# lreithmayr/ORB_SLAM2_2021

Hardware: AMD Instinct MI355X
Metric: frames/sec (ORB extract+match) on 1241×376, 1/2/4/8 MI355X; % HBM roofline (higher is better)
Workload: dtype u8

## Files before the change

orb_slam2_2021_amd/csrc/orbfe_extract.hip:

```cpp
#include <hip/hip_runtime.h>

#include <algorithm>
#include <atomic>
#include <chrono>
#include <condition_variable>
#include <functional>
#include <thread>
#include <cfloat>
#include <cmath>
#include <cstdio>
#include <cstdlib>
#include <cstring>
#include <mutex>
#include <string>
#include <type_traits>
#include <vector>

#include "../../include/orbfe.h"
#include "../../include/orbfe_debug.h"
#include "orb_pattern31.inc"
#include "orbfe_device.h"
#include "orbfe_internal.h"
#include "orbfe_ktimer.h"

// ... 1004 lines not shown
        const int m = mp[0];
        const int mn = max(max(max(max((int)mp[-mw - 1], (int)mp[-mw]), max((int)mp[-mw + 1], (int)mp[-1])),
                               max(max((int)mp[1], (int)mp[mw - 1]), (int)mp[mw])), (int)mp[mw + 1]);
        sc = m - 1;
        keep = m >= max(t + 1, 2) && m > mn;
      }
      const uint64_t bal = wave_ballot(keep);
      if (keep) out[count + prefix_in_wave(bal)] = pack_key(cc + 3 + cd.ox, rr + 3 + cd.oy, sc);
      count += __popcll(bal);
    }
    if (count > 0) break;
  }
  if (lane == 0) *cnt_out = count;
}

#define OCT_MISC_SCALAR 16
#define OCT_MISC_INTS 32
struct ONode {
  int16_t x0, y0, x1, y1;
  int32_t begin, count, seq, flags;
};


__device__ __forceinline__ int child_of(uint32_t key, int mx, int my) {
  return (key_x(key) >= mx ? 1 : 0) | (key_y(key) >= my ? 2 : 0);
}

__device__ __forceinline__ int4 wave_child_counts(const ONode& nd, const uint32_t* ka, const uint32_t* kb) {
  const uint32_t* src = (nd.flags & 1) ? kb : ka;
  const int mx = nd.x0 + ((nd.x1 - nd.x0 + 1) >> 1), my = nd.y0 + ((nd.y1 - nd.y0 + 1) >> 1);
  int c0 = 0, c1 = 0, c2 = 0, c3 = 0;
  for (int i0 = 0; i0 < nd.count; i0 += 64) {
    const int i = i0 + lane_id();
    const int ch = i < nd.count ? child_of(src[nd.begin + i], mx, my) : -1;
    c0 += __popcll(wave_ballot(ch == 0));
    c1 += __popcll(wave_ballot(ch == 1));
    c2 += __popcll(wave_ballot(ch == 2));
    c3 += __popcll(wave_ballot(ch == 3));
  }
  return make_int4(c0, c1, c2, c3);
}

__device__ __forceinline__ void wave_child_partition(const ONode& nd, int4 cnt, uint32_t* ka, uint32_t* kb) {
  const uint32_t* src = (nd.flags & 1) ? kb : ka;
  uint32_t* dst = (nd.flags & 1) ? ka : kb;
  const int mx = nd.x0 + ((nd.x1 - nd.x0 + 1) >> 1), my = nd.y0 + ((nd.y1 - nd.y0 + 1) >> 1);
  int o0 = nd.begin, o1 = o0 + cnt.x, o2 = o1 + cnt.y, o3 = o2 + cnt.z;
  for (int i0 = 0; i0 < nd.count; i0 += 64) {
    const int i = i0 + lane_id();
    uint32_t key = 0;
    int ch = -1;
    if (i < nd.count) {
      key = src[nd.begin + i];
      ch = child_of(key, mx, my);
    }
    const uint64_t b0 = wave_ballot(ch == 0), b1 = wave_ballot(ch == 1), b2 = wave_ballot(ch == 2),
                   b3 = wave_ballot(ch == 3);
    if (ch == 0) dst[o0 + prefix_in_wave(b0)] = key;
    if (ch == 1) dst[o1 + prefix_in_wave(b1)] = key;
    if (ch == 2) dst[o2 + prefix_in_wave(b2)] = key;
    if (ch == 3) dst[o3 + prefix_in_wave(b3)] = key;
    o0 += __popcll(b0);
    o1 += __popcll(b1);
    o2 += __popcll(b2);
    o3 += __popcll(b3);
  }
}

#ifndef OCT_SMALL
#define OCT_SMALL 48
#endif
#define OCT_SMALL_MAX 128
__device__ __forceinline__ int4 serial_child_counts(const ONode& nd, const uint32_t* ka, const uint32_t* kb) {
  const uint32_t* src = ((nd.flags & 1) ? kb : ka) + nd.begin;
  const int mx = nd.x0 + ((nd.x1 - nd.x0 + 1) >> 1), my = nd.y0 + ((nd.y1 - nd.y0 + 1) >> 1);
  uint32_t c = 0;
  if (nd.count <= 16) {
    uint32_t key[16];
#pragma unroll
    for (int j = 0; j < 16; j++) key[j] = j < nd.count ? src[j] : 0u;
#pragma unroll
    for (int j = 0; j < 16; j++)
      if (j < nd.count) c += 1u << (8 * child_of(key[j], mx, my));
    return make_int4((int)(c & 255u), (int)((c >> 8) & 255u), (int)((c >> 16) & 255u), (int)(c >> 24));
  }
  int i = 0;
  for (; i + 4 <= nd.count; i += 4) {
    const uint32_t k0 = src[i], k1 = src[i + 1], k2 = src[i + 2], k3 = src[i + 3];
    c += (1u << (8 * child_of(k0, mx, my))) + (1u << (8 * child_of(k1, mx, my))) +
         (1u << (8 * child_of(k2, mx, my))) + (1u << (8 * child_of(k3, mx, my)));
  }
  for (; i < nd.count; i++) c += 1u << (8 * child_of(src[i], mx, my));
  return make_int4((int)(c & 255u), (int)((c >> 8) & 255u), (int)((c >> 16) & 255u), (int)(c >> 24));
}

__device__ __forceinline__ void serial_child_partition(const ONode& nd, int4 cnt, uint32_t* ka, uint32_t* kb) {
  const uint32_t* src = ((nd.flags & 1) ? kb : ka) + nd.begin;
  uint32_t* dst = ((nd.flags & 1) ? ka : kb) + nd.begin;
  const int mx = nd.x0 + ((nd.x1 - nd.x0 + 1) >> 1), my = nd.y0 + ((nd.y1 - nd.y0 + 1) >> 1);
  uint32_t o = ((uint32_t)cnt.x << 8) | ((uint32_t)(cnt.x + cnt.y) << 16) | ((uint32_t)(cnt.x + cnt.y + cnt.z) << 24);
  auto put = [&](uint32_t key) {
    const int sh = 8 * child_of(key, mx, my);
    dst[(o >> sh) & 255u] = key;
    o += 1u << sh;
  };
  if (nd.count <= 16) {
    uint32_t key[16];
#pragma unroll
    for (int j = 0; j < 16; j++) key[j] = j < nd.count ? src[j] : 0u;
#pragma unroll
    for (int j = 0; j < 16; j++)
      if (j < nd.count) put(key[j]);
    return;
  }
  int i = 0;
  for (; i + 4 <= nd.count; i += 4) {
    const uint32_t k0 = src[i], k1 = src[i + 1], k2 = src[i + 2], k3 = src[i + 3];
    put(k0);
    put(k1);
    put(k2);
    put(k3);
  }
  for (; i < nd.count; i++) put(src[i]);
}

#define OCT_WJ 16
#define OCT_SJ 16
__device__ __forceinline__ int4 wave_child_split(const ONode& nd, uint32_t* ka, uint32_t* kb) {
  if (nd.count > 64 * OCT_WJ) {
    const int4 c4 = wave_child_counts(nd, ka, kb);
    wave_child_partition(nd, c4, ka, kb);
    return c4;
  }
  const uint32_t* src = ((nd.flags & 1) ? kb : ka) + nd.begin;
  uint32_t* dst = ((nd.flags & 1) ? ka : kb) + nd.begin;
  const int mx = nd.x0 + ((nd.x1 - nd.x0 + 1) >> 1), my = nd.y0 + ((nd.y1 - nd.y0 + 1) >> 1);
  const int lane = lane_id();
  uint32_t key[OCT_WJ];
  int ch[OCT_WJ];
#pragma unroll
  for (int j = 0; j < OCT_WJ; j++) {
    const int i = 64 * j + lane;
    key[j] = i < nd.count ? src[i] : 0u;
  }
  int c0 = 0, c1 = 0, c2 = 0, c3 = 0;
#pragma unroll
  for (int j = 0; j < OCT_WJ; j++) {
    if (64 * j >= nd.count) break;
    ch[j] = 64 * j + lane < nd.count ? child_of(key[j], mx, my) : -1;
    c0 += __popcll(wave_ballot(ch[j] == 0));
    c1 += __popcll(wave_ballot(ch[j] == 1));
    c2 += __popcll(wave_ballot(ch[j] == 2));
    c3 += __popcll(wave_ballot(ch[j] == 3));
  }
  int o0 = 0, o1 = c0, o2 = c0 + c1, o3 = c0 + c1 + c2;
#pragma unroll
  for (int j = 0; j < OCT_WJ; j++) {
    if (64 * j >= nd.count) break;
    const uint64_t b0 = wave_ballot(ch[j] == 0), b1 = wave_ballot(ch[j] == 1), b2 = wave_ballot(ch[j] == 2),
                   b3 = wave_ballot(ch[j] == 3);
    if (ch[j] == 0) dst[o0 + prefix_in_wave(b0)] = key[j];
    if (ch[j] == 1) dst[o1 + prefix_in_wave(b1)] = key[j];
    if (ch[j] == 2) dst[o2 + prefix_in_wave(b2)] = key[j];
    if (ch[j] == 3) dst[o3 + prefix_in_wave(b3)] = key[j];
    o0 += __popcll(b0);
    o1 += __popcll(b1);
    o2 += __popcll(b2);
    o3 += __popcll(b3);
  }
  return make_int4(c0, c1, c2, c3);
}

__device__ __forceinline__ int4 serial_child_split(const ONode& nd, uint32_t* ka, uint32_t* kb) {
  if (nd.count > OCT_SJ) {
    const int4 c4 = serial_child_counts(nd, ka, kb);
    serial_child_partition(nd, c4, ka, kb);
    return c4;
  }
  const uint32_t* src = ((nd.flags & 1) ? kb : ka) + nd.begin;
  uint32_t* dst = ((nd.flags & 1) ? ka : kb) + nd.begin;
  const int mx = nd.x0 + ((nd.x1 - nd.x0 + 1) >> 1), my = nd.y0 + ((nd.y1 - nd.y0 + 1) >> 1);
  uint32_t key[OCT_SJ];
#pragma unroll
  for (int j = 0; j < OCT_SJ; j++) key[j] = j < nd.count ? src[j] : 0u;
  uint32_t c = 0;
#pragma unroll
  for (int j = 0; j < OCT_SJ; j++)
    if (j < nd.count) c += 1u << (8 * child_of(key[j], mx, my));
  const uint32_t c0 = c & 255u, c1 = (c >> 8) & 255u, c2 = (c >> 16) & 255u;
  uint32_t o = (c0 << 8) | ((c0 + c1) << 16) | ((c0 + c1 + c2) << 24);
#pragma unroll
  for (int j = 0; j < OCT_SJ; j++)
    if (j < nd.count) {
      const int sh = 8 * child_of(key[j], mx, my);
      dst[(o >> sh) & 255u] = key[j];
      o += 1u << sh;
    }
  return make_int4((int)c0, (int)c1, (int)c2, (int)(c >> 24));
}

__device__ __forceinline__ ONode make_child(const ONode& p, int c, int begin, int count, int seq) {
  const int mx = p.x0 + ((p.x1 - p.x0 + 1) >> 1), my = p.y0 + ((p.y1 - p.y0 + 1) >> 1);
  ONode n;
  n.x0 = (int16_t)((c & 1) ? mx : p.x0);
  n.x1 = (int16_t)((c & 1) ? p.x1 : mx);
  n.y0 = (int16_t)((c & 2) ? my : p.y0);
  n.y1 = (int16_t)((c & 2) ? p.y1 : my);
  n.begin = begin;
  n.count = count;
  n.seq = seq;
  n.flags = ((p.flags & 1) ^ 1) | (count > 1 ? 2 : 0);
  return n;
}

__device__ __forceinline__ int nonempty4(int4 c) {
  return (c.x > 0) + (c.y > 0) + (c.z > 0) + (c.w > 0);
}
__device__ __forceinline__ int multi4(int4 c) {
  return (c.x > 1) + (c.y > 1) + (c.z > 1) + (c.w > 1);
}
__device__ __forceinline__ int comp4(int4 c, int k) {
  return k == 0 ? c.x : k == 1 ? c.y : k == 2 ? c.z : c.w;
}

template <int NW, typename Idx, typename F>
__device__ __forceinline__ void for_big_nodes(const ONode* L, int m, int small, Idx idx, F f) {
  const int w = wave_id(), lane = lane_id();
  int ord = 0;
  for (int c0 = 0; c0 < m; c0 += 64) {
    const int p = c0 + lane;
    const bool big = p < m && L[idx(p)].count > small;
    uint64_t bal = wave_ballot(big);
    while (bal) {
      const int b = __builtin_ctzll(bal);
      bal &= bal - 1;
      if (ord % NW == w) f(c0 + b);
      ord++;
    }
  }
}

#ifdef ORBFE_OCT_PROF
__device__ unsigned long long g_oct_prof[64 * 16 * 16];
#define OCT_MARK(k, v) \
  do { if (threadIdx.x == 0 && blockIdx.y < 64 && l < 16) g_oct_prof[(blockIdx.y * 16 + l) * 16 + (k)] = (v); } while (0)
#else
#define OCT_MARK(k, v) do { } while (0)
#endif
#ifdef ORBFE_OCT_PROF_PASS
#define OCT_RMARK(k, v) do { } while (0)
#define OCT_PMARK(k, v) do { if (n_passes == ORBFE_OCT_PROF_PASS) OCT_MARK(k, v); } while (0)
#else
#define OCT_RMARK(k, v) OCT_MARK(k, v)
#define OCT_PMARK(k, v) do { } while (0)
#endif

template <bool LDSK, int NT>
__device__ __forceinline__ void octree_run(const ExtractArgs& a, uint8_t* smem, int l, int n, uint32_t* ka,
                                           uint32_t* kb) {
  constexpr int NW = NT / 64;
  const int img = blockIdx.y;
  const int t = threadIdx.x, w = wave_id(), lane = lane_id();
  const int NC = a.node_cap, SC = a.sort_cap, SA = a.scan_cap;
  const int SMALL = a.oct_small;
  ONode* nodes0 = reinterpret_cast<ONode*>(smem);
  ONode* nodes1 = nodes0 + NC;
  int4* cc = reinterpret_cast<int4*>(nodes1 + NC);
  int* sa = reinterpret_cast<int*>(cc + NC);
  int* sb = sa + SA;
  int* sx = sb + SA;
  unsigned long long* sk = reinterpret_cast<unsigned long long*>(sx + SA);
  int* misc = reinterpret_cast<int*>(sk + SC);
  const LevelDesc ld = a.levels[l];
  const int N = ld.budget;
  const uint32_t* cand = a.cand + (long long)img * a.cand_stride;
  uint32_t* out = a.lvlkeys + (long long)img * a.lvlkey_stride + ld.key_begin;
  int32_t* out_n = a.lvlcnt + (long long)img * a.nlevels + l;

  const int ncells = ld.ncells;
  for (int c = t; c < ncells; c += NT) {
    const int b0 = sa[c], cnt = (c + 1 < ncells ? sa[c + 1] : n) - b0;
    const uint32_t* src = cand + sx[c];
    int k = 0;
    for (; k + 4 <= cnt; k += 4) {
      const uint32_t v0 = src[k], v1 = src[k + 1], v2 = src[k + 2], v3 = src[k + 3];
      ka[b0 + k] = v0;
      ka[b0 + k + 1] = v1;
      ka[b0 + k + 2] = v2;
      ka[b0 + k + 3] = v3;
    }
    for (; k < cnt; k++) ka[b0 + k] = src[k];
  }
  __syncthreads();
  OCT_MARK(2, wall_clock64());

  const int nini = ld.nini;
  const float hx = ld.hx;
  auto ini_node = [&](uint32_t key) -> int {
    const int x = key_x(key);
    if (nini > 8) return (int)((float)x / hx);
    int b = 0;
#pragma unroll
    for (int k = 1; k < 8; k++) b += (k < nini && x >= ld.ini_thr[k]) ? 1 : 0;
    return b;
  };
  int* bcnt = reinterpret_cast<int*>(sk);
  int* boff = bcnt + NW * nini;
  const int R = ((n + NW - 1) / NW + 63) & ~63;
  const int wbeg = min(w * R, n), wend = min(wbeg + R, n);
  constexpr int INI_J = NT >= 1024 ? 8 : 24;
  const bool cached = wend - wbeg <= 64 * INI_J;
  uint32_t kr[INI_J];
  int br[INI_J];
  const int nj = (wend - wbeg + 63) >> 6;
  if (cached) {
#pragma unroll
    for (int j = 0; j < INI_J; j++) br[j] = -1;
    if (nini <= 8) {
#pragma unroll
      for (int j = 0; j < INI_J; j++) {
        if (j >= nj) break;
        const int i = wbeg + 64 * j + lane;
        kr[j] = i < wend ? ka[i] : 0u;
        const int x = key_x(kr[j]);
        int b = 0;
#pragma unroll
// ... 84 lines not shown
    }
  }
  __syncthreads();
  if (t == 0) {
    int S = 0, run = 0;
    for (int b = 0; b < nini; b++) {
      const int cnt = sb[b];
      if (cnt > 0) {
        ONode nd;
        nd.x0 = (int16_t)(int)(hx * (float)b);
        nd.x1 = (int16_t)(int)(hx * (float)(b + 1));
        nd.y0 = 0;
        nd.y1 = (int16_t)ld.rel_h;
        nd.begin = run;
        nd.count = cnt;
        nd.seq = b;
        nd.flags = 1;
        nodes0[S++] = nd;
      }
      run += cnt;
    }
    misc[OCT_MISC_SCALAR] = S;
  }
  __syncthreads();

  int S = misc[OCT_MISC_SCALAR];
  int cur = 0;
  bool refine = false;
  OCT_MARK(3, wall_clock64());
  int n_passes = 0, n_rounds = 0;
  for (int iter = 0; iter < 4 * NC + 64; iter++) {
    ONode* Lc = cur ? nodes1 : nodes0;
    ONode* Ln = cur ? nodes0 : nodes1;
    const int prevS = S;
    if (!refine) {
      n_passes++;
#ifdef ORBFE_OCT_PROF_PASS
      if (n_passes == ORBFE_OCT_PROF_PASS) OCT_MARK(14, wall_clock64());
#endif
      for (int i = t; i < S; i += NT) {
        const ONode nd = Lc[i];
        if (nd.count > SMALL) continue;
        const bool par = nd.count > 1;
        const int4 c4 = par ? serial_child_split(nd, ka, kb) : make_int4(0, 0, 0, 0);
        if (par) cc[i] = c4;
        sa[i] = par ? nonempty4(c4) : 0;
        sb[i] = par ? 0 : 1;
        sx[i] = par ? multi4(c4) : 0;
      }
      OCT_PMARK(8, wall_clock64());
#ifdef ORBFE_OCT_PROF_PASS
      unsigned long long split_cyc = 0, split_n = 0;
#endif
      for_big_nodes<NW>(Lc, S, SMALL, [](int p) { return p; }, [&](int i) {
#ifdef ORBFE_OCT_PROF_PASS
        const unsigned long long c0 = clock64();
        const int4 c4 = wave_child_split(Lc[i], ka, kb);
        split_cyc += clock64() - c0;
        split_n += (unsigned long long)Lc[i].count << 16 | 1ull;
#else
        const int4 c4 = wave_child_split(Lc[i], ka, kb);
#endif
        if (lane == 0) {
          cc[i] = c4;
          sa[i] = nonempty4(c4);
          sb[i] = 0;
          sx[i] = multi4(c4);
        }
      });
      OCT_PMARK(9, wall_clock64());
#ifdef ORBFE_OCT_PROF_PASS
      OCT_PMARK(12, split_cyc);
      OCT_PMARK(13, split_n);
#endif
      __syncthreads();
      OCT_PMARK(10, wall_clock64());
#ifndef ORBFE_OCT_PROF_PASS
      if (n_passes == 1) OCT_MARK(14, wall_clock64());
#endif
      const int3 tot3 = block_scan_excl3_n<NT>(sa, sb, sx, S, reinterpret_cast<int*>(sk));
#ifndef ORBFE_OCT_PROF_PASS
      if (n_passes == 1) OCT_MARK(15, wall_clock64());
#endif
      OCT_PMARK(11, wall_clock64());
      const int T = tot3.x, NP = tot3.y, nexp = tot3.z;
      for (int i = t; i < S; i += NT) {
        const ONode nd = Lc[i];
        if (nd.count > 1) {
          const int4 c4 = cc[i];
          int e = sa[i], off = nd.begin;
          for (int k = 0; k < 4; k++) {
            const int ck = comp4(c4, k);
            if (ck > 0) {
              Ln[T - 1 - e] = make_child(nd, k, off, ck, e);
              e++;
            }
            off += ck;
          }
        } else {
          ONode m = nd;
          m.flags &= 1;
          Ln[T + sb[i]] = m;
        }
      }
      S = T + NP;
      cur ^= 1;
      __syncthreads();
#ifdef ORBFE_OCT_PROF_PASS
      if (n_passes == ORBFE_OCT_PROF_PASS) OCT_MARK(15, wall_clock64());
#endif
      if (S >= N || S == prevS) break;
      if (S + nexp * 3 > N) refine = true;
    } else {
      if (n_rounds++ == 0) OCT_MARK(4, wall_clock64());
      for (int i = t; i < S; i += NT) sa[i] = (Lc[i].flags & 2) ? 1 : 0;
      __syncthreads();
      const int nR = block_scan_excl_n<NT>(sa, S, misc);
      if (n_rounds == 1) OCT_RMARK(8, wall_clock64());
      int P2 = 1;
      while (P2 < nR) P2 <<= 1;
      if (nR > 1024) {
        for (int i = t; i < P2; i += NT) sk[i] = 0ull;
        __syncthreads();
      }
      for (int i = t; i < S; i += NT) {
        const ONode nd = Lc[i];
        if (nd.flags & 2)
          sk[sa[i]] = ((unsigned long long)nd.count << 40) | ((unsigned long long)nd.seq << 20) |
                      (unsigned long long)i;
      }
      __syncthreads();
      if (nR <= 1024) {
        constexpr int RP = (1024 + NT - 1) / NT;
        unsigned long long kk[RP];
        int rk[RP];
#pragma unroll
        for (int r = 0; r < RP; r++) {
          const int k = t + NT * r;
          kk[r] = k < nR ? sk[k] : 0ull;
          rk[r] = 0;
        }
        const int per = (nR + NT - 1) / NT;
        int j = 0;
// ... 25 lines not shown
            for (int pidx = t; pidx < (P2 >> 1); pidx += NT) {
              const int i = ((pidx & ~(j - 1)) << 1) | (pidx & (j - 1)), ixj = i + j;
              const unsigned long long x = sk[i], y = sk[ixj];
              if ((i & k) == 0 ? (x < y) : (x > y)) {
                sk[i] = y;
                sk[ixj] = x;
              }
            }
            __syncthreads();
          }
        }
      }
      if (n_rounds == 1) OCT_RMARK(9, wall_clock64());
      for (int k = t; k < nR; k += NT) {
        const ONode nd = Lc[(int)(sk[k] & 0xfffffull)];
        if (nd.count <= SMALL) cc[k] = serial_child_counts(nd, ka, kb);
      }
      for_big_nodes<NW>(Lc, nR, SMALL, [&](int k) { return (int)(sk[k] & 0xfffffull); }, [&](int k) {
        const int4 c4 = wave_child_counts(Lc[(int)(sk[k] & 0xfffffull)], ka, kb);
        if (lane == 0) cc[k] = c4;
      });
      __syncthreads();
      if (n_rounds == 1) OCT_RMARK(10, wall_clock64());
      for (int k = t; k < nR; k += NT) sa[k] = nonempty4(cc[k]) - 1;
      if (t == 0) misc[OCT_MISC_SCALAR + 1] = nR;
      __syncthreads();
      block_scan_excl_n<NT>(sa, nR, misc);
      for (int k = t; k < nR; k += NT) {
        const int incl = sa[k] + nonempty4(cc[k]) - 1;
        if (prevS + incl >= N) atomicMin(&misc[OCT_MISC_SCALAR + 1], k + 1);
      }
      __syncthreads();
      const int nproc = misc[OCT_MISC_SCALAR + 1];
      if (n_rounds == 1) OCT_RMARK(11, wall_clock64());
      for (int i = t; i < S; i += NT) sb[i] = -1;
      __syncthreads();
      for (int k = t; k < nproc; k += NT) sb[(int)(sk[k] & 0xfffffull)] = k;
      __syncthreads();
      for (int k = t; k < nproc; k += NT) {
        const ONode nd = Lc[(int)(sk[k] & 0xfffffull)];
        if (nd.count <= SMALL) serial_child_partition(nd, cc[k], ka, kb);
      }
      for_big_nodes<NW>(Lc, nproc, SMALL, [&](int k) { return (int)(sk[k] & 0xfffffull); }, [&](int k) {
        wave_child_partition(Lc[(int)(sk[k] & 0xfffffull)], cc[k], ka, kb);
      });
      for (int k = t; k < nR; k += NT) sx[k] = k < nproc ? nonempty4(cc[k]) : 0;
      __syncthreads();
      if (n_rounds == 1) OCT_RMARK(12, wall_clock64());
      const int T = block_scan_excl_n<NT>(sx, nR, misc);
      for (int i = t; i < S; i += NT) sa[i] = sb[i] < 0 ? 1 : 0;
      __syncthreads();
      const int NK = block_scan_excl_n<NT>(sa, S, misc);
      for (int i = t; i < S; i += NT) {
        const ONode nd = Lc[i];
        const int k = sb[i];
        if (k >= 0) {
          const int4 c4 = cc[k];
          int e = sx[k], off = nd.begin;
          for (int c = 0; c < 4; c++) {
            const int ck = comp4(c4, c);
            if (ck > 0) {
              Ln[T - 1 - e] = make_child(nd, c, off, ck, e);
              e++;
            }
            off += ck;
          }
        } else {
          ONode m = nd;
          m.flags &= 1;
          Ln[T + sa[i]] = m;
        }
      }
      S = T + NK;
      cur ^= 1;
      __syncthreads();
      if (n_rounds == 1) OCT_RMARK(13, wall_clock64());
      if (S >= N || S == prevS) break;
    }
  }

  OCT_MARK(5, wall_clock64());
  if (n_rounds == 0) OCT_MARK(4, wall_clock64());
  ONode* Lf = cur ? nodes1 : nodes0;
  for (int i = t; i < S; i += NT) {
    const ONode nd = Lf[i];
    const uint32_t* src = (nd.flags & 1) ? kb : ka;
    uint32_t best = src[nd.begin];
    for (int k = 1; k < nd.count; k++) {
      const uint32_t key = src[nd.begin + k];
      if (key_s(key) > key_s(best)) best = key;
    }
    out[i] = pack_key(key_x(best) + 16, key_y(best) + 16, key_s(best));
  }
  if (t == 0) *out_n = S;
#ifdef ORBFE_OCT_PROF
  __syncthreads();
  OCT_MARK(6, wall_clock64());
  OCT_MARK(7, (unsigned long long)n | ((unsigned long long)n_passes << 24) | ((unsigned long long)n_rounds << 32) |
                  ((unsigned long long)S << 48));
#endif
}


template <int NT>
__global__ __launch_bounds__(NT) void k_octree(ExtractArgs a, int l0) {
  extern __shared__ __attribute__((aligned(16))) uint8_t smem[];
  const int l = l0 + blockIdx.x, img = blockIdx.y, t = threadIdx.x;
  const int NC = a.node_cap, SC = a.sort_cap, SA = a.scan_cap;
  int* sa = reinterpret_cast<int*>(smem + (sizeof(ONode) * 2 + sizeof(int4)) * NC);
  int* sx = sa + 2 * SA;
  int* misc = reinterpret_cast<int*>(reinterpret_cast<unsigned long long*>(sx + SA) + SC);
  uint32_t* lds_keys = reinterpret_cast<uint32_t*>(misc + OCT_MISC_INTS);
  OCT_MARK(0, wall_clock64());
  const LevelDesc ld = a.levels[l];
  const int32_t* ccount = a.cellcnt + (long long)img * a.ncells + ld.cell_begin;
  for (int c = t; c < ld.ncells; c += NT) {
    sa[c] = ccount[c];
    sx[c] = a.cells[ld.cell_begin + c].slot;
  }
  __syncthreads();
  const int n = block_scan_excl_n<NT>(sa, ld.ncells, misc);
  OCT_MARK(1, wall_clock64());
  if (n == 0) {
    if (t == 0) a.lvlcnt[(long long)img * a.nlevels + l] = 0;
    return;
  }
  if (n <= a.key_lds_cap) {
    octree_run<true, NT>(a, smem, l, n, lds_keys, lds_keys + a.key_lds_cap);
  } else {
    octree_run<false, NT>(a, smem, l, n, a.keys_a + (long long)img * a.keyscr_stride + ld.cand_begin,
                      a.keys_b + (long long)img * a.keyscr_stride + ld.cand_begin);
  }
}

#define BS_W 248
#define BS_H 16
__device__ __forceinline__ int reflect101(int i, int n) {
  return i < 0 ? -i : (i >= n ? 2 * n - 2 - i : i);
}

__device__ __forceinline__ uint32_t from_left(uint32_t v) {
  return (uint32_t)__builtin_amdgcn_mov_dpp((int)v, 0x138, 0xf, 0xf, true);
}
__device__ __forceinline__ uint32_t from_right(uint32_t v) {
  return (uint32_t)__builtin_amdgcn_mov_dpp((int)v, 0x130, 0xf, 0xf, true);
}
// ... 786 lines not shown
    }
  }
  return ORBFE_OK;
}

static OctPlan octree_plan(const std::vector<LevelDesc>& lv, int l0, int l1, int budget_kb, int key_cap_override) {
  OctPlan p;
  if (l1 <= l0) return p;
  int ncap = 0, mc = 0, mini = 0;
  for (int l = l0; l < l1; l++) {
    ncap = std::max(ncap, lv[l].key_cap + 4);
    mc = std::max(mc, lv[l].ncells);
    mini = std::max(mini, lv[l].nini);
  }
  int sc = 1;
  while (sc < std::max(std::max(ncap, 16 * mini), 24)) sc <<= 1;
  p.node_cap = ncap;
  p.sort_cap = sc;
  p.scan_cap = (std::max(ncap, mc) + 3) & ~3;
  const size_t fixed = sizeof(ONode) * 2 * ncap + sizeof(int4) * ncap + sizeof(int) * 3 * p.scan_cap +
                       sizeof(unsigned long long) * sc + sizeof(int) * OCT_MISC_INTS;
  const size_t budget = (size_t)budget_kb * 1024;
  p.key_lds_cap = fixed < budget ? (int)((budget - fixed) / 8) & ~63 : 0;
  if (key_cap_override >= 0) p.key_lds_cap = std::min(p.key_lds_cap, key_cap_override);
  p.lds = fixed + sizeof(uint32_t) * 2 * (size_t)p.key_lds_cap;
  return p;
}

static void free_batch(orbfe_extractor* h) {
  if (h->hpyr_pending) {
    hipEventSynchronize(h->ev_hpyr);
    h->hpyr_pending = false;
  }
  drop_graphs(h);
  hipFree(h->d_pyr);
  hipFree(h->d_blur);
  hipFree(h->d_cand);
  hipFree(h->d_cellcnt);
  hipFree(h->d_keys_a);
  hipFree(h->d_keys_b);
// ... 243 lines not shown
    hipEvent_t e = nullptr;
    ORBFE_HIP_CHECK(hipEventCreateWithFlags(&e, kForkJoinEvent));
    h->ev_lvl.push_back(e);
  }
  hipStreamCaptureStatus cs = hipStreamCaptureStatusNone;
  if (!h->use_graphs || !st || h->side_ext || orbfe_kt::g_on.load(std::memory_order_relaxed) ||
      hipStreamIsCapturing(st, &cs) != hipSuccess || cs != hipStreamCaptureStatusNone)
    return launch_extract(h, n, d_imgs, img_stride, pitch, d_kps, d_desc, cap, d_counts, st, i0);
  const hipStream_t side = h->inline_side ? st : (h->side_ext ? h->side_ext : h->side);
  const std::vector<uintptr_t> key = {
      (uintptr_t)n, (uintptr_t)d_imgs, (uintptr_t)img_stride, (uintptr_t)pitch, (uintptr_t)d_kps,
      (uintptr_t)d_desc, (uintptr_t)cap, (uintptr_t)d_counts, (uintptr_t)st, (uintptr_t)i0, (uintptr_t)side,
      (uintptr_t)h->rows, (uintptr_t)h->cols, (uintptr_t)h->geom_mode, (uintptr_t)h->d_levels,
      (uintptr_t)h->d_pyr, (uintptr_t)h->d_blur, (uintptr_t)h->d_cand, (uintptr_t)h->d_cellcnt,
      (uintptr_t)h->d_keys_a, (uintptr_t)h->d_keys_b, (uintptr_t)h->d_lvlkeys, (uintptr_t)h->d_lvlcnt,
      (uintptr_t)h->key_lds_cap, (uintptr_t)h->octree_split, (uintptr_t)(h->oct_hi_kb * 1024 + h->oct_lo_kb), (uintptr_t)h->device_call, (uintptr_t)(h->fast_wpb_side * 16 + h->fast_wpb_main), (uintptr_t)h->fast_side_levels, (uintptr_t)h->fast_side_merge, (uintptr_t)h->input_l0, (uintptr_t)h->inline_side, (uintptr_t)(h->oct_threads_small * 4096 + h->oct_threads_batch), (uintptr_t)h->pyr_small.d_tiles, (uintptr_t)h->pyr_batch.d_tiles,
      (uintptr_t)h->blur_mode};
  h->graph_clock++;
  hipGraphExec_t exec = nullptr;
  for (auto& e : h->graphs)
    if (e.key == key) {
      exec = e.exec;
      e.used = h->graph_clock;
      h->graph_hits++;
      break;
    }
  if (!exec) {
    hipGraph_t g = nullptr;
    ORBFE_HIP_CHECK(hipStreamBeginCapture(st, hipStreamCaptureModeThreadLocal));
    const int r = launch_extract(h, n, d_imgs, img_stride, pitch, d_kps, d_desc, cap, d_counts, st, i0);
    const hipError_t ee = hipStreamEndCapture(st, &g);
// ... 936 lines not shown
  h->pyr_tiles_small[0] = small_tx;
  h->pyr_tiles_small[1] = small_ty;
  h->pyr_tiles_batch[0] = batch_tx;
  h->pyr_tiles_batch[1] = batch_ty;
  h->rows = h->cols = -1;
  drop_graphs(h);
  return ORBFE_OK;
}

extern "C" int orbfe_debug_set_octree_threads(orbfe_extractor* h, int small_calls, int batches) {
  auto ok = [](int t) { return t == 256 || t == 512 || t == 1024; };
  if (!h || !ok(small_calls) || !ok(batches))
    return orbfe_set_error(ORBFE_ERR_ARG, "orbfe_debug_set_octree_threads: 256, 512 or 1024");
  h->oct_threads_small = small_calls;
  h->oct_threads_batch = batches;
  return ORBFE_OK;
}

extern "C" int orbfe_debug_set_octree_threads_l0(orbfe_extractor* h, int threads) {
  if (!h || !(threads == 0 || threads == 256 || threads == 512 || threads == 1024))
    return orbfe_set_error(ORBFE_ERR_ARG, "orbfe_debug_set_octree_threads_l0: 0, 256, 512 or 1024");
  h->oct_threads_l0 = threads;
  return ORBFE_OK;
}

extern "C" int orbfe_debug_set_octree_serial(orbfe_extractor* h, int small_calls, int batches) {
  if (!h || small_calls < 1 || small_calls > OCT_SMALL_MAX || batches < 1 || batches > OCT_SMALL_MAX)
    return orbfe_set_error(ORBFE_ERR_ARG, "orbfe_debug_set_octree_serial: 1 .. 128 keys");
  h->oct_small_small = small_calls;
  h->oct_small_batch = batches;
  drop_graphs(h);
  return ORBFE_OK;
}

extern "C" int orbfe_debug_set_latency_schedule(orbfe_extractor* h, int k) {
  if (!h) return orbfe_set_error(ORBFE_ERR_ARG, "orbfe_debug_set_latency_schedule: null handle");
  h->lat_sched = k > 0 ? k : 0;
// ... 43 lines not shown
```

Baseline: 87000.

## Partition octree keys in place with a single LDS key buffer

The octree split now partitions keys in place within one buffer instead of ping-ponging between two buffers. Large nodes stage through a global scratch buffer and copy back. Node structs drop their seq/flags fields, and child counts are packed into 64-bit words. The sort keys alias the next node list, and a new 16-lane group split handles mid-sized nodes. The aim is to halve the LDS needed for keys so more levels keep their keys on-chip, and to spread mid-size node work across lanes. The cost is an extra copy-back for big nodes and more complex LDS aliasing.

```diff
diff --git a/orb_slam2_2021_amd/csrc/orbfe_extract.hip b/orb_slam2_2021_amd/csrc/orbfe_extract.hip
--- a/orb_slam2_2021_amd/csrc/orbfe_extract.hip
+++ b/orb_slam2_2021_amd/csrc/orbfe_extract.hip
@@ -1042,25 +1042,55 @@
   if (lane == 0) *cnt_out = count;
 }
 
-#define OCT_MISC_SCALAR 16
-#define OCT_MISC_INTS 32
+#define OCT_MISC_SCALAR 48
+#define OCT_MISC_INTS 64
 struct ONode {
   int16_t x0, y0, x1, y1;
-  int32_t begin, count, seq, flags;
+  int32_t begin, count;
 };
 
+__device__ __forceinline__ unsigned long long pack_cc(int4 c) {
+  return (unsigned long long)c.x | ((unsigned long long)c.y << 21) | ((unsigned long long)c.z << 42);
+}
+__device__ __forceinline__ int4 unpack_cc(unsigned long long v, int count) {
+  const int x = (int)(v & 0x1fffffull), y = (int)((v >> 21) & 0x1fffffull), z = (int)(v >> 42);
+  return make_int4(x, y, z, count - x - y - z);
+}
+
+struct OctLds {
+  ONode *nodes0, *nodes1;
+  unsigned long long* cc;
+  int *sa, *sb, *sx, *misc;
+  uint32_t* keys;
+};
+__host__ __device__ __forceinline__ size_t oct_list_bytes(int node_cap, int sort_cap) {
+  const size_t nb = sizeof(ONode) * (size_t)node_cap, sb = sizeof(unsigned long long) * (size_t)sort_cap;
+  return ((nb > sb ? nb : sb) + 15) & ~(size_t)15;
+}
+__device__ __forceinline__ OctLds oct_lds(uint8_t* smem, int NC, int SC, int SA) {
+  OctLds o;
+  const size_t lb = oct_list_bytes(NC, SC);
+  o.nodes0 = reinterpret_cast<ONode*>(smem);
+  o.nodes1 = reinterpret_cast<ONode*>(smem + lb);
+  o.cc = reinterpret_cast<unsigned long long*>(smem + 2 * lb);
+  o.sa = reinterpret_cast<int*>(o.cc + NC);
+  o.sb = o.sa + SA;
+  o.sx = o.sb + SA;
+  o.misc = o.sx + SA;
+  o.keys = reinterpret_cast<uint32_t*>(o.misc + OCT_MISC_INTS);
+  return o;
+}
 
 __device__ __forceinline__ int child_of(uint32_t key, int mx, int my) {
   return (key_x(key) >= mx ? 1 : 0) | (key_y(key) >= my ? 2 : 0);
 }
 
-__device__ __forceinline__ int4 wave_child_counts(const ONode& nd, const uint32_t* ka, const uint32_t* kb) {
-  const uint32_t* src = (nd.flags & 1) ? kb : ka;
+__device__ __forceinline__ int4 wave_child_counts(const ONode& nd, const uint32_t* k) {
   const int mx = nd.x0 + ((nd.x1 - nd.x0 + 1) >> 1), my = nd.y0 + ((nd.y1 - nd.y0 + 1) >> 1);
   int c0 = 0, c1 = 0, c2 = 0, c3 = 0;
   for (int i0 = 0; i0 < nd.count; i0 += 64) {
     const int i = i0 + lane_id();
-    const int ch = i < nd.count ? child_of(src[nd.begin + i], mx, my) : -1;
+    const int ch = i < nd.count ? child_of(k[nd.begin + i], mx, my) : -1;
     c0 += __popcll(wave_ballot(ch == 0));
     c1 += __popcll(wave_ballot(ch == 1));
     c2 += __popcll(wave_ballot(ch == 2));
@@ -1069,9 +1099,7 @@
   return make_int4(c0, c1, c2, c3);
 }
 
-__device__ __forceinline__ void wave_child_partition(const ONode& nd, int4 cnt, uint32_t* ka, uint32_t* kb) {
-  const uint32_t* src = (nd.flags & 1) ? kb : ka;
-  uint32_t* dst = (nd.flags & 1) ? ka : kb;
+__device__ __forceinline__ void wave_child_partition_staged(const ONode& nd, int4 cnt, uint32_t* k, uint32_t* g) {
   const int mx = nd.x0 + ((nd.x1 - nd.x0 + 1) >> 1), my = nd.y0 + ((nd.y1 - nd.y0 + 1) >> 1);
   int o0 = nd.begin, o1 = o0 + cnt.x, o2 = o1 + cnt.y, o3 = o2 + cnt.z;
   for (int i0 = 0; i0 < nd.count; i0 += 64) {
@@ -1079,28 +1107,40 @@
     uint32_t key = 0;
     int ch = -1;
     if (i < nd.count) {
-      key = src[nd.begin + i];
+      key = k[nd.begin + i];
       ch = child_of(key, mx, my);
     }
     const uint64_t b0 = wave_ballot(ch == 0), b1 = wave_ballot(ch == 1), b2 = wave_ballot(ch == 2),
                    b3 = wave_ballot(ch == 3);
-    if (ch == 0) dst[o0 + prefix_in_wave(b0)] = key;
-    if (ch == 1) dst[o1 + prefix_in_wave(b1)] = key;
-    if (ch == 2) dst[o2 + prefix_in_wave(b2)] = key;
-    if (ch == 3) dst[o3 + prefix_in_wave(b3)] = key;
+    if (ch == 0) g[o0 + prefix_in_wave(b0)] = key;
+    if (ch == 1) g[o1 + prefix_in_wave(b1)] = key;
+    if (ch == 2) g[o2 + prefix_in_wave(b2)] = key;
+    if (ch == 3) g[o3 + prefix_in_wave(b3)] = key;
     o0 += __popcll(b0);
     o1 += __popcll(b1);
     o2 += __popcll(b2);
     o3 += __popcll(b3);
   }
+  __threadfence_block();
+  __builtin_amdgcn_wave_barrier();
+  int i = lane_id();
+  for (; i + 192 < nd.count; i += 256) {
+    const uint32_t v0 = g[nd.begin + i], v1 = g[nd.begin + i + 64], v2 = g[nd.begin + i + 128],
+                   v3 = g[nd.begin + i + 192];
+    k[nd.begin + i] = v0;
+    k[nd.begin + i + 64] = v1;
+    k[nd.begin + i + 128] = v2;
+    k[nd.begin + i + 192] = v3;
+  }
+  for (; i < nd.count; i += 64) k[nd.begin + i] = g[nd.begin + i];
 }
 
 #ifndef OCT_SMALL
 #define OCT_SMALL 48
 #endif
 #define OCT_SMALL_MAX 128
-__device__ __forceinline__ int4 serial_child_counts(const ONode& nd, const uint32_t* ka, const uint32_t* kb) {
-  const uint32_t* src = ((nd.flags & 1) ? kb : ka) + nd.begin;
+__device__ __forceinline__ int4 serial_child_counts(const ONode& nd, const uint32_t* k) {
+  const uint32_t* src = k + nd.begin;
   const int mx = nd.x0 + ((nd.x1 - nd.x0 + 1) >> 1), my = nd.y0 + ((nd.y1 - nd.y0 + 1) >> 1);
   uint32_t c = 0;
   if (nd.count <= 16) {
@@ -1122,46 +1162,16 @@
   return make_int4((int)(c & 255u), (int)((c >> 8) & 255u), (int)((c >> 16) & 255u), (int)(c >> 24));
 }
 
-__device__ __forceinline__ void serial_child_partition(const ONode& nd, int4 cnt, uint32_t* ka, uint32_t* kb) {
-  const uint32_t* src = ((nd.flags & 1) ? kb : ka) + nd.begin;
-  uint32_t* dst = ((nd.flags & 1) ? ka : kb) + nd.begin;
-  const int mx = nd.x0 + ((nd.x1 - nd.x0 + 1) >> 1), my = nd.y0 + ((nd.y1 - nd.y0 + 1) >> 1);
-  uint32_t o = ((uint32_t)cnt.x << 8) | ((uint32_t)(cnt.x + cnt.y) << 16) | ((uint32_t)(cnt.x + cnt.y + cnt.z) << 24);
-  auto put = [&](uint32_t key) {
-    const int sh = 8 * child_of(key, mx, my);
-    dst[(o >> sh) & 255u] = key;
-    o += 1u << sh;
-  };
-  if (nd.count <= 16) {
-    uint32_t key[16];
-#pragma unroll
-    for (int j = 0; j < 16; j++) key[j] = j < nd.count ? src[j] : 0u;
-#pragma unroll
-    for (int j = 0; j < 16; j++)
-      if (j < nd.count) put(key[j]);
-    return;
-  }
-  int i = 0;
-  for (; i + 4 <= nd.count; i += 4) {
-    const uint32_t k0 = src[i], k1 = src[i + 1], k2 = src[i + 2], k3 = src[i + 3];
-    put(k0);
-    put(k1);
-    put(k2);
-    put(k3);
-  }
-  for (; i < nd.count; i++) put(src[i]);
-}
-
 #define OCT_WJ 16
+#define OCT_GJ 8
 #define OCT_SJ 16
-__device__ __forceinline__ int4 wave_child_split(const ONode& nd, uint32_t* ka, uint32_t* kb) {
+__device__ __forceinline__ int4 wave_child_split(const ONode& nd, uint32_t* k, uint32_t* g) {
   if (nd.count > 64 * OCT_WJ) {
-    const int4 c4 = wave_child_counts(nd, ka, kb);
-    wave_child_partition(nd, c4, ka, kb);
+    const int4 c4 = wave_child_counts(nd, k);
+    wave_child_partition_staged(nd, c4, k, g);
     return c4;
   }
-  const uint32_t* src = ((nd.flags & 1) ? kb : ka) + nd.begin;
-  uint32_t* dst = ((nd.flags & 1) ? ka : kb) + nd.begin;
+  uint32_t* seg = k + nd.begin;
   const int mx = nd.x0 + ((nd.x1 - nd.x0 + 1) >> 1), my = nd.y0 + ((nd.y1 - nd.y0 + 1) >> 1);
   const int lane = lane_id();
   uint32_t key[OCT_WJ];
@@ -1169,7 +1179,7 @@
 #pragma unroll
   for (int j = 0; j < OCT_WJ; j++) {
     const int i = 64 * j + lane;
-    key[j] = i < nd.count ? src[i] : 0u;
+    key[j] = i < nd.count ? seg[i] : 0u;
   }
   int c0 = 0, c1 = 0, c2 = 0, c3 = 0;
 #pragma unroll
@@ -1187,10 +1197,10 @@
     if (64 * j >= nd.count) break;
     const uint64_t b0 = wave_ballot(ch[j] == 0), b1 = wave_ballot(ch[j] == 1), b2 = wave_ballot(ch[j] == 2),
                    b3 = wave_ballot(ch[j] == 3);
-    if (ch[j] == 0) dst[o0 + prefix_in_wave(b0)] = key[j];
-    if (ch[j] == 1) dst[o1 + prefix_in_wave(b1)] = key[j];
-    if (ch[j] == 2) dst[o2 + prefix_in_wave(b2)] = key[j];
-    if (ch[j] == 3) dst[o3 + prefix_in_wave(b3)] = key[j];
+    if (ch[j] == 0) seg[o0 + prefix_in_wave(b0)] = key[j];
+    if (ch[j] == 1) seg[o1 + prefix_in_wave(b1)] = key[j];
+    if (ch[j] == 2) seg[o2 + prefix_in_wave(b2)] = key[j];
+    if (ch[j] == 3) seg[o3 + prefix_in_wave(b3)] = key[j];
     o0 += __popcll(b0);
     o1 += __popcll(b1);
     o2 += __popcll(b2);
@@ -1199,18 +1209,55 @@
   return make_int4(c0, c1, c2, c3);
 }
 
-__device__ __forceinline__ int4 serial_child_split(const ONode& nd, uint32_t* ka, uint32_t* kb) {
-  if (nd.count > OCT_SJ) {
-    const int4 c4 = serial_child_counts(nd, ka, kb);
-    serial_child_partition(nd, c4, ka, kb);
-    return c4;
-  }
-  const uint32_t* src = ((nd.flags & 1) ? kb : ka) + nd.begin;
-  uint32_t* dst = ((nd.flags & 1) ? ka : kb) + nd.begin;
+__device__ __forceinline__ int4 group_child_split(const ONode& nd, bool on, uint32_t* k) {
+  const int lane = lane_id(), gl = lane & 15, gsh = lane & 48;
+  const int count = on ? nd.count : 0;
+  uint32_t* seg = k + nd.begin;
+  const int mx = nd.x0 + ((nd.x1 - nd.x0 + 1) >> 1), my = nd.y0 + ((nd.y1 - nd.y0 + 1) >> 1);
+  uint32_t key[OCT_GJ];
+  int ch[OCT_GJ];
+#pragma unroll
+  for (int j = 0; j < OCT_GJ; j++) {
+    const int i = 16 * j + gl;
+    key[j] = i < count ? seg[i] : 0u;
+    ch[j] = i < count ? child_of(key[j], mx, my) : -1;
+  }
+  const uint32_t below = (1u << gl) - 1u;
+  int c0 = 0, c1 = 0, c2 = 0, c3 = 0;
+#pragma unroll
+  for (int j = 0; j < OCT_GJ; j++) {
+    if (wave_ballot(16 * j < count) == 0) break;
+    c0 += __popc((uint32_t)(wave_ballot(ch[j] == 0) >> gsh) & 0xffffu);
+    c1 += __popc((uint32_t)(wave_ballot(ch[j] == 1) >> gsh) & 0xffffu);
+    c2 += __popc((uint32_t)(wave_ballot(ch[j] == 2) >> gsh) & 0xffffu);
+    c3 += __popc((uint32_t)(wave_ballot(ch[j] == 3) >> gsh) & 0xffffu);
+  }
+  int o0 = 0, o1 = c0, o2 = c0 + c1, o3 = c0 + c1 + c2;
+#pragma unroll
+  for (int j = 0; j < OCT_GJ; j++) {
+    if (wave_ballot(16 * j < count) == 0) break;
+    const uint32_t b0 = (uint32_t)(wave_ballot(ch[j] == 0) >> gsh) & 0xffffu,
+                   b1 = (uint32_t)(wave_ballot(ch[j] == 1) >> gsh) & 0xffffu,
+                   b2 = (uint32_t)(wave_ballot(ch[j] == 2) >> gsh) & 0xffffu,
+                   b3 = (uint32_t)(wave_ballot(ch[j] == 3) >> gsh) & 0xffffu;
+    if (ch[j] == 0) seg[o0 + __popc(b0 & below)] = key[j];
+    if (ch[j] == 1) seg[o1 + __popc(b1 & below)] = key[j];
+    if (ch[j] == 2) seg[o2 + __popc(b2 & below)] = key[j];
+    if (ch[j] == 3) seg[o3 + __popc(b3 & below)] = key[j];
+    o0 += __popc(b0);
+    o1 += __popc(b1);
+    o2 += __popc(b2);
+    o3 += __popc(b3);
+  }
+  return make_int4(c0, c1, c2, c3);
+}
+
+__device__ __forceinline__ int4 serial_child_split(const ONode& nd, uint32_t* k) {
+  uint32_t* seg = k + nd.begin;
   const int mx = nd.x0 + ((nd.x1 - nd.x0 + 1) >> 1), my = nd.y0 + ((nd.y1 - nd.y0 + 1) >> 1);
   uint32_t key[OCT_SJ];
 #pragma unroll
-  for (int j = 0; j < OCT_SJ; j++) key[j] = j < nd.count ? src[j] : 0u;
+  for (int j = 0; j < OCT_SJ; j++) key[j] = j < nd.count ? seg[j] : 0u;
   uint32_t c = 0;
 #pragma unroll
   for (int j = 0; j < OCT_SJ; j++)
@@ -1221,13 +1268,13 @@
   for (int j = 0; j < OCT_SJ; j++)
     if (j < nd.count) {
       const int sh = 8 * child_of(key[j], mx, my);
-      dst[(o >> sh) & 255u] = key[j];
+      seg[(o >> sh) & 255u] = key[j];
       o += 1u << sh;
     }
   return make_int4((int)c0, (int)c1, (int)c2, (int)(c >> 24));
 }
 
-__device__ __forceinline__ ONode make_child(const ONode& p, int c, int begin, int count, int seq) {
+__device__ __forceinline__ ONode make_child(const ONode& p, int c, int begin, int count) {
   const int mx = p.x0 + ((p.x1 - p.x0 + 1) >> 1), my = p.y0 + ((p.y1 - p.y0 + 1) >> 1);
   ONode n;
   n.x0 = (int16_t)((c & 1) ? mx : p.x0);
@@ -1236,8 +1283,6 @@
   n.y1 = (int16_t)((c & 2) ? p.y1 : my);
   n.begin = begin;
   n.count = count;
-  n.seq = seq;
-  n.flags = ((p.flags & 1) ^ 1) | (count > 1 ? 2 : 0);
   return n;
 }
 
@@ -1264,6 +1309,24 @@
       bal &= bal - 1;
       if (ord % NW == w) f(c0 + b);
       ord++;
+    }
+  }
+}
+
+template <int NW, typename Idx, typename F>
+__device__ __forceinline__ void for_mid_nodes(const ONode* L, int m, int lo, int hi, Idx idx, F f) {
+  const int w = wave_id(), lane = lane_id(), g = lane >> 4;
+  for (int c0 = 0; c0 < m; c0 += 64) {
+    const int p = c0 + lane;
+    const int cnt = p < m ? L[idx(p)].count : 0;
+    const bool mid = cnt > lo && cnt <= hi;
+    const uint64_t bal = wave_ballot(mid);
+    const int nmid = __popcll(bal), rank = prefix_in_wave(bal);
+    for (int base = 4 * w; base < nmid; base += 4 * NW) {
+      const uint64_t m0 = wave_ballot(mid && rank == base), m1 = wave_ballot(mid && rank == base + 1),
+                     m2 = wave_ballot(mid && rank == base + 2), m3 = wave_ballot(mid && rank == base + 3);
+      const uint64_t mine = g == 0 ? m0 : g == 1 ? m1 : g == 2 ? m2 : m3;
+      f(c0 + (mine ? __builtin_ctzll(mine) : 0), mine != 0);
     }
   }
 }
@@ -1284,27 +1347,28 @@
 #endif
 
 template <bool LDSK, int NT>
-__device__ __forceinline__ void octree_run(const ExtractArgs& a, uint8_t* smem, int l, int n, uint32_t* ka,
-                                           uint32_t* kb) {
+__device__ __forceinline__ void octree_run(const ExtractArgs& a, uint8_t* smem, int l, int n, uint32_t* kb,
+                                           uint32_t* gs) {
   constexpr int NW = NT / 64;
   const int img = blockIdx.y;
   const int t = threadIdx.x, w = wave_id(), lane = lane_id();
-  const int NC = a.node_cap, SC = a.sort_cap, SA = a.scan_cap;
-  const int SMALL = a.oct_small;
-  ONode* nodes0 = reinterpret_cast<ONode*>(smem);
-  ONode* nodes1 = nodes0 + NC;
-  int4* cc = reinterpret_cast<int4*>(nodes1 + NC);
-  int* sa = reinterpret_cast<int*>(cc + NC);
-  int* sb = sa + SA;
-  int* sx = sb + SA;
-  unsigned long long* sk = reinterpret_cast<unsigned long long*>(sx + SA);
-  int* misc = reinterpret_cast<int*>(sk + SC);
+  const int NC = a.node_cap;
+  const int SMALL = a.oct_small, SER = min(SMALL, OCT_SJ);
+  const OctLds o = oct_lds(smem, NC, a.sort_cap, a.scan_cap);
+  ONode *nodes0 = o.nodes0, *nodes1 = o.nodes1;
+  unsigned long long* cc = o.cc;
+  int *sa = o.sa, *sb = o.sb, *sx = o.sx;
+  int* misc = o.misc;
   const LevelDesc ld = a.levels[l];
   const int N = ld.budget;
   const uint32_t* cand = a.cand + (long long)img * a.cand_stride;
   uint32_t* out = a.lvlkeys + (long long)img * a.lvlkey_stride + ld.key_begin;
   int32_t* out_n = a.lvlcnt + (long long)img * a.nlevels + l;
 
+  constexpr int INI_J = NT >= 1024 ? 8 : 24;
+  const int R = ((n + NW - 1) / NW + 63) & ~63;
+  const bool cached = R <= 64 * INI_J;
+  uint32_t* ka = cached ? kb : gs;
   const int ncells = ld.ncells;
   for (int c = t; c < ncells; c += NT) {
     const int b0 = sa[c], cnt = (c + 1 < ncells ? sa[c + 1] : n) - b0;
@@ -1332,12 +1396,9 @@
     for (int k = 1; k < 8; k++) b += (k < nini && x >= ld.ini_thr[k]) ? 1 : 0;
     return b;
   };
-  int* bcnt = reinterpret_cast<int*>(sk);
+  int* bcnt = reinterpret_cast<int*>(nodes1);
   int* boff = bcnt + NW * nini;
-  const int R = ((n + NW - 1) / NW + 63) & ~63;
   const int wbeg = min(w * R, n), wend = min(wbeg + R, n);
-  constexpr int INI_J = NT >= 1024 ? 8 : 24;
-  const bool cached = wend - wbeg <= 64 * INI_J;
   uint32_t kr[INI_J];
   int br[INI_J];
   const int nj = (wend - wbeg + 63) >> 6;
@@ -1452,8 +1513,6 @@
         nd.y1 = (int16_t)ld.rel_h;
         nd.begin = run;
         nd.count = cnt;
-        nd.seq = b;
-        nd.flags = 1;
         nodes0[S++] = nd;
       }
       run += cnt;
@@ -1464,12 +1523,14 @@
 
   int S = misc[OCT_MISC_SCALAR];
   int cur = 0;
+  int lastT = 0;
   bool refine = false;
   OCT_MARK(3, wall_clock64());
   int n_passes = 0, n_rounds = 0;
   for (int iter = 0; iter < 4 * NC + 64; iter++) {
     ONode* Lc = cur ? nodes1 : nodes0;
     ONode* Ln = cur ? nodes0 : nodes1;
+    unsigned long long* sk = reinterpret_cast<unsigned long long*>(Ln);
     const int prevS = S;
     if (!refine) {
       n_passes++;
@@ -1478,14 +1539,23 @@
 #endif
       for (int i = t; i < S; i += NT) {
         const ONode nd = Lc[i];
-        if (nd.count > SMALL) continue;
+        if (nd.count > SER) continue;
         const bool par = nd.count > 1;
-        const int4 c4 = par ? serial_child_split(nd, ka, kb) : make_int4(0, 0, 0, 0);
-        if (par) cc[i] = c4;
+        const int4 c4 = par ? serial_child_split(nd, kb) : make_int4(0, 0, 0, 0);
+        if (par) cc[i] = pack_cc(c4);
         sa[i] = par ? nonempty4(c4) : 0;
         sb[i] = par ? 0 : 1;
         sx[i] = par ? multi4(c4) : 0;
       }
+      for_mid_nodes<NW>(Lc, S, SER, SMALL, [](int p) { return p; }, [&](int i, bool on) {
+        const int4 c4 = group_child_split(Lc[i], on, kb);
+        if (on && (lane & 15) == 0) {
+          cc[i] = pack_cc(c4);
+          sa[i] = nonempty4(c4);
+          sb[i] = 0;
+          sx[i] = multi4(c4);
+        }
+      });
       OCT_PMARK(8, wall_clock64());
 #ifdef ORBFE_OCT_PROF_PASS
       unsigned long long split_cyc = 0, split_n = 0;
@@ -1493,14 +1563,14 @@
       for_big_nodes<NW>(Lc, S, SMALL, [](int p) { return p; }, [&](int i) {
 #ifdef ORBFE_OCT_PROF_PASS
         const unsigned long long c0 = clock64();
-        const int4 c4 = wave_child_split(Lc[i], ka, kb);
+        const int4 c4 = wave_child_split(Lc[i], kb, gs);
         split_cyc += clock64() - c0;
         split_n += (unsigned long long)Lc[i].count << 16 | 1ull;
 #else
-        const int4 c4 = wave_child_split(Lc[i], ka, kb);
+        const int4 c4 = wave_child_split(Lc[i], kb, gs);
 #endif
         if (lane == 0) {
-          cc[i] = c4;
+          cc[i] = pack_cc(c4);
           sa[i] = nonempty4(c4);
           sb[i] = 0;
           sx[i] = multi4(c4);
@@ -1516,7 +1586,7 @@
 #ifndef ORBFE_OCT_PROF_PASS
       if (n_passes == 1) OCT_MARK(14, wall_clock64());
 #endif
-      const int3 tot3 = block_scan_excl3_n<NT>(sa, sb, sx, S, reinterpret_cast<int*>(sk));
+      const int3 tot3 = block_scan_excl3_n<NT>(sa, sb, sx, S, misc);
 #ifndef ORBFE_OCT_PROF_PASS
       if (n_passes == 1) OCT_MARK(15, wall_clock64());
 #endif
@@ -1525,23 +1595,22 @@
       for (int i = t; i < S; i += NT) {
         const ONode nd = Lc[i];
         if (nd.count > 1) {
-          const int4 c4 = cc[i];
+          const int4 c4 = unpack_cc(cc[i], nd.count);
           int e = sa[i], off = nd.begin;
           for (int k = 0; k < 4; k++) {
             const int ck = comp4(c4, k);
             if (ck > 0) {
-              Ln[T - 1 - e] = make_child(nd, k, off, ck, e);
+              Ln[T - 1 - e] = make_child(nd, k, off, ck);
               e++;
             }
             off += ck;
           }
         } else {
-          ONode m = nd;
-          m.flags &= 1;
-          Ln[T + sb[i]] = m;
+          Ln[T + sb[i]] = nd;
         }
       }
       S = T + NP;
+      lastT = T;
       cur ^= 1;
       __syncthreads();
 #ifdef ORBFE_OCT_PROF_PASS
@@ -1551,7 +1620,7 @@
       if (S + nexp * 3 > N) refine = true;
     } else {
       if (n_rounds++ == 0) OCT_MARK(4, wall_clock64());
-      for (int i = t; i < S; i += NT) sa[i] = (Lc[i].flags & 2) ? 1 : 0;
+      for (int i = t; i < S; i += NT) sa[i] = (i < lastT && Lc[i].count > 1) ? 1 : 0;
       __syncthreads();
       const int nR = block_scan_excl_n<NT>(sa, S, misc);
       if (n_rounds == 1) OCT_RMARK(8, wall_clock64());
@@ -1563,8 +1632,8 @@
       }
       for (int i = t; i < S; i += NT) {
         const ONode nd = Lc[i];
-        if (nd.flags & 2)
-          sk[sa[i]] = ((unsigned long long)nd.count << 40) | ((unsigned long long)nd.seq << 20) |
+        if (i < lastT && nd.count > 1)
+          sk[sa[i]] = ((unsigned long long)nd.count << 40) | ((unsigned long long)(lastT - 1 - i) << 20) |
                       (unsigned long long)i;
       }
       __syncthreads();
@@ -1620,20 +1689,27 @@
       if (n_rounds == 1) OCT_RMARK(9, wall_clock64());
       for (int k = t; k < nR; k += NT) {
         const ONode nd = Lc[(int)(sk[k] & 0xfffffull)];
-        if (nd.count <= SMALL) cc[k] = serial_child_counts(nd, ka, kb);
+        if (nd.count <= SMALL) {
+          const int4 c4 = serial_child_counts(nd, kb);
+          cc[k] = pack_cc(c4);
+          sx[k] = nonempty4(c4);
+        }
       }
       for_big_nodes<NW>(Lc, nR, SMALL, [&](int k) { return (int)(sk[k] & 0xfffffull); }, [&](int k) {
-        const int4 c4 = wave_child_counts(Lc[(int)(sk[k] & 0xfffffull)], ka, kb);
-        if (lane == 0) cc[k] = c4;
+        const int4 c4 = wave_child_counts(Lc[(int)(sk[k] & 0xfffffull)], kb);
+        if (lane == 0) {
+          cc[k] = pack_cc(c4);
+          sx[k] = nonempty4(c4);
+        }
       });
       __syncthreads();
       if (n_rounds == 1) OCT_RMARK(10, wall_clock64());
-      for (int k = t; k < nR; k += NT) sa[k] = nonempty4(cc[k]) - 1;
+      for (int k = t; k < nR; k += NT) sa[k] = sx[k] - 1;
       if (t == 0) misc[OCT_MISC_SCALAR + 1] = nR;
       __syncthreads();
       block_scan_excl_n<NT>(sa, nR, misc);
       for (int k = t; k < nR; k += NT) {
-        const int incl = sa[k] + nonempty4(cc[k]) - 1;
+        const int incl = sa[k] + sx[k] - 1;
         if (prevS + incl >= N) atomicMin(&misc[OCT_MISC_SCALAR + 1], k + 1);
       }
       __syncthreads();
@@ -1645,12 +1721,16 @@
       __syncthreads();
       for (int k = t; k < nproc; k += NT) {
         const ONode nd = Lc[(int)(sk[k] & 0xfffffull)];
-        if (nd.count <= SMALL) serial_child_partition(nd, cc[k], ka, kb);
-      }
+        if (nd.count <= SER) serial_child_split(nd, kb);
+      }
+      for_mid_nodes<NW>(Lc, nproc, SER, SMALL, [&](int k) { return (int)(sk[k] & 0xfffffull); }, [&](int k, bool on) {
+        group_child_split(Lc[(int)(sk[k] & 0xfffffull)], on, kb);
+      });
       for_big_nodes<NW>(Lc, nproc, SMALL, [&](int k) { return (int)(sk[k] & 0xfffffull); }, [&](int k) {
-        wave_child_partition(Lc[(int)(sk[k] & 0xfffffull)], cc[k], ka, kb);
+        wave_child_split(Lc[(int)(sk[k] & 0xfffffull)], kb, gs);
       });
-      for (int k = t; k < nR; k += NT) sx[k] = k < nproc ? nonempty4(cc[k]) : 0;
+      for (int k = t; k < nR; k += NT)
+        if (k >= nproc) sx[k] = 0;
       __syncthreads();
       if (n_rounds == 1) OCT_RMARK(12, wall_clock64());
       const int T = block_scan_excl_n<NT>(sx, nR, misc);
@@ -1661,23 +1741,22 @@
         const ONode nd = Lc[i];
         const int k = sb[i];
         if (k >= 0) {
-          const int4 c4 = cc[k];
+          const int4 c4 = unpack_cc(cc[k], nd.count);
           int e = sx[k], off = nd.begin;
           for (int c = 0; c < 4; c++) {
             const int ck = comp4(c4, c);
             if (ck > 0) {
-              Ln[T - 1 - e] = make_child(nd, c, off, ck, e);
+              Ln[T - 1 - e] = make_child(nd, c, off, ck);
               e++;
             }
             off += ck;
           }
         } else {
-          ONode m = nd;
-          m.flags &= 1;
-          Ln[T + sa[i]] = m;
+          Ln[T + sa[i]] = nd;
         }
       }
       S = T + NK;
+      lastT = T;
       cur ^= 1;
       __syncthreads();
       if (n_rounds == 1) OCT_RMARK(13, wall_clock64());
@@ -1690,7 +1769,7 @@
   ONode* Lf = cur ? nodes1 : nodes0;
   for (int i = t; i < S; i += NT) {
     const ONode nd = Lf[i];
-    const uint32_t* src = (nd.flags & 1) ? kb : ka;
+    const uint32_t* src = kb;
     uint32_t best = src[nd.begin];
     for (int k = 1; k < nd.count; k++) {
       const uint32_t key = src[nd.begin + k];
@@ -1712,11 +1791,8 @@
 __global__ __launch_bounds__(NT) void k_octree(ExtractArgs a, int l0) {
   extern __shared__ __attribute__((aligned(16))) uint8_t smem[];
   const int l = l0 + blockIdx.x, img = blockIdx.y, t = threadIdx.x;
-  const int NC = a.node_cap, SC = a.sort_cap, SA = a.scan_cap;
-  int* sa = reinterpret_cast<int*>(smem + (sizeof(ONode) * 2 + sizeof(int4)) * NC);
-  int* sx = sa + 2 * SA;
-  int* misc = reinterpret_cast<int*>(reinterpret_cast<unsigned long long*>(sx + SA) + SC);
-  uint32_t* lds_keys = reinterpret_cast<uint32_t*>(misc + OCT_MISC_INTS);
+  const OctLds o = oct_lds(smem, a.node_cap, a.sort_cap, a.scan_cap);
+  int *sa = o.sa, *sx = o.sx, *misc = o.misc;
   OCT_MARK(0, wall_clock64());
   const LevelDesc ld = a.levels[l];
   const int32_t* ccount = a.cellcnt + (long long)img * a.ncells + ld.cell_begin;
@@ -1731,11 +1807,11 @@
     if (t == 0) a.lvlcnt[(long long)img * a.nlevels + l] = 0;
     return;
   }
+  uint32_t* gs = a.keys_a + (long long)img * a.keyscr_stride + ld.cand_begin;
   if (n <= a.key_lds_cap) {
-    octree_run<true, NT>(a, smem, l, n, lds_keys, lds_keys + a.key_lds_cap);
+    octree_run<true, NT>(a, smem, l, n, o.keys, gs);
   } else {
-    octree_run<false, NT>(a, smem, l, n, a.keys_a + (long long)img * a.keyscr_stride + ld.cand_begin,
-                      a.keys_b + (long long)img * a.keyscr_stride + ld.cand_begin);
+    octree_run<false, NT>(a, smem, l, n, a.keys_b + (long long)img * a.keyscr_stride + ld.cand_begin, gs);
   }
 }
 
@@ -2552,16 +2628,17 @@
     mini = std::max(mini, lv[l].nini);
   }
   int sc = 1;
-  while (sc < std::max(std::max(ncap, 16 * mini), 24)) sc <<= 1;
+  while (sc < std::max(ncap, 16 * mini)) sc <<= 1;
   p.node_cap = ncap;
   p.sort_cap = sc;
   p.scan_cap = (std::max(ncap, mc) + 3) & ~3;
-  const size_t fixed = sizeof(ONode) * 2 * ncap + sizeof(int4) * ncap + sizeof(int) * 3 * p.scan_cap +
-                       sizeof(unsigned long long) * sc + sizeof(int) * OCT_MISC_INTS;
+  const size_t scratch = 0;
+  const size_t fixed = 2 * oct_list_bytes(ncap, sc) + sizeof(unsigned long long) * ncap +
+                       sizeof(int) * 3 * p.scan_cap + sizeof(int) * OCT_MISC_INTS + scratch;
   const size_t budget = (size_t)budget_kb * 1024;
-  p.key_lds_cap = fixed < budget ? (int)((budget - fixed) / 8) & ~63 : 0;
+  p.key_lds_cap = fixed < budget ? (int)((budget - fixed) / 4) & ~63 : 0;
   if (key_cap_override >= 0) p.key_lds_cap = std::min(p.key_lds_cap, key_cap_override);
-  p.lds = fixed + sizeof(uint32_t) * 2 * (size_t)p.key_lds_cap;
+  p.lds = fixed + sizeof(uint32_t) * (size_t)p.key_lds_cap;
   return p;
 }
 
@@ -2835,7 +2912,7 @@
       (uintptr_t)h->rows, (uintptr_t)h->cols, (uintptr_t)h->geom_mode, (uintptr_t)h->d_levels,
       (uintptr_t)h->d_pyr, (uintptr_t)h->d_blur, (uintptr_t)h->d_cand, (uintptr_t)h->d_cellcnt,
       (uintptr_t)h->d_keys_a, (uintptr_t)h->d_keys_b, (uintptr_t)h->d_lvlkeys, (uintptr_t)h->d_lvlcnt,
-      (uintptr_t)h->key_lds_cap, (uintptr_t)h->octree_split, (uintptr_t)(h->oct_hi_kb * 1024 + h->oct_lo_kb), (uintptr_t)h->device_call, (uintptr_t)(h->fast_wpb_side * 16 + h->fast_wpb_main), (uintptr_t)h->fast_side_levels, (uintptr_t)h->fast_side_merge, (uintptr_t)h->input_l0, (uintptr_t)h->inline_side, (uintptr_t)(h->oct_threads_small * 4096 + h->oct_threads_batch), (uintptr_t)h->pyr_small.d_tiles, (uintptr_t)h->pyr_batch.d_tiles,
+      (uintptr_t)h->key_lds_cap, (uintptr_t)h->octree_split, (uintptr_t)(h->oct_hi_kb * 1024 + h->oct_lo_kb), (uintptr_t)h->device_call, (uintptr_t)(h->fast_wpb_side * 16 + h->fast_wpb_main), (uintptr_t)h->fast_side_levels, (uintptr_t)h->fast_side_merge, (uintptr_t)h->input_l0, (uintptr_t)h->inline_side, (uintptr_t)(h->oct_threads_small * 4096 + h->oct_threads_batch), (uintptr_t)(h->oct_threads_l0 * 2 + (h->call_inline ? 1 : 0)), (uintptr_t)h->pyr_small.d_tiles, (uintptr_t)h->pyr_batch.d_tiles,
       (uintptr_t)h->blur_mode};
   h->graph_clock++;
   hipGraphExec_t exec = nullptr;
@@ -3802,6 +3879,7 @@
     return orbfe_set_error(ORBFE_ERR_ARG, "orbfe_debug_set_octree_threads: 256, 512 or 1024");
   h->oct_threads_small = small_calls;
   h->oct_threads_batch = batches;
+  drop_graphs(h);
   return ORBFE_OK;
 }
 
@@ -3809,6 +3887,7 @@
   if (!h || !(threads == 0 || threads == 256 || threads == 512 || threads == 1024))
     return orbfe_set_error(ORBFE_ERR_ARG, "orbfe_debug_set_octree_threads_l0: 0, 256, 512 or 1024");
   h->oct_threads_l0 = threads;
+  drop_graphs(h);
   return ORBFE_OK;
 }
 
```

After: 87060 (median of 3 runs). Within noise of the previous version (+0.1%).
